# zrlhahaha/Direct12PBRRenderer

Measured on AMD Instinct MI355X. Metric: shaded Mpixel/s at 4K G-buffer (full deferred frame: clustered shade + bloom + auto-exposure + ACES), higher is better.
Workload: dtype f32

## Files before the change

direct12pbrrenderer_amd/csrc/bloom.hip:

```cpp
#include <type_traits>
#include "pbr_internal.hpp"
#include "pbr_device.hpp"

using namespace pbr;

__constant__ float c_gauss[9] = {0.0148f, 0.0459f, 0.1050f, 0.1941f, 0.2803f, 0.1941f, 0.1050f, 0.0459f, 0.0148f};

__device__ __forceinline__ float4 to4(F4 v) { return make_float4(v.x, v.y, v.z, v.w); }
__device__ __forceinline__ F4 from4(float4 v) { return f4(v.x, v.y, v.z, v.w); }

struct OutRect { int x0, y0, x1, y1, ox, oy, pitch; };
constexpr int PF_MAX_RECTS = 5;
struct OutRects {
    int n, ox, oy, pitch;
    int x0[PF_MAX_RECTS], y0[PF_MAX_RECTS], x1[PF_MAX_RECTS], y1[PF_MAX_RECTS], tiles_x[PF_MAX_RECTS], first[PF_MAX_RECTS + 1];
};
__device__ __forceinline__ float4 soft_knee_sample(F4 c, float threshold, float knee) {
    const float brightness = fmaxf(c.x, fmaxf(c.y, c.z));
    float soft = fminf(fmaxf(brightness - threshold + threshold * knee, 0.0f), 2.0f * threshold * knee);
    soft /= 4.0f * threshold * knee + 0.00001f;
    const float contribution = fmaxf(soft, brightness - threshold) / fmaxf(brightness, 0.00001f);
    const float cr = c.x * contribution, cg = c.y * contribution, cb = c.z * contribution;
    const float wgt = 1.0f / (luminance(cr, cg, cb) + 1.0f);
    return make_float4(cr * wgt, cg * wgt, cb * wgt, wgt);
// ... 377 lines not shown
    static_assert(SR % NW == 0 && TH % NW == 0 && PER_T * 8 <= 64, "rows must split evenly over the waves; one halo tap per lane");
    __shared__ float4 sLine[DUAL ? 2 : 1][NW][SW];
    __shared__ H4 sT[SR][TW];
    __shared__ uint32_t sh_hist[TAIL == 2 ? NW : 1][TAIL == 2 ? PBR_HISTOGRAM_BINS : 1];
    const int t = threadIdx.x, lane = t & 63;
    const int wv = __builtin_amdgcn_readfirstlane(t >> 6);
    if (TAIL == 2) hist_clear<NT>(sh_hist, t);
    const LevelAlpha alpha = level_alpha<MODE, DUAL>(in, iw, ih, in2, ow, oh, tr);
    for (int tile = blockIdx.x; tile < n_tiles; tile += gridDim.x) {
    const int x0 = (tr.tx0 + tile % tiles_x) * TW, y0 = (tr.ty0 + tile / tiles_x) * TH;
    const int x = x0 + lane;
    H4 hdr_in[PER_O];
    const bool in_mx = TAIL != 0 && merge_has_x(tr, x);
    if (TAIL != 0) {
#pragma unroll
        for (int k = 0; k < PER_O; k++) {
            const int y = y0 + wv + NW * k;
            if (merge_has(tr, in_mx, y)) hdr_in[k] = *reinterpret_cast<const H4*>(out + 4 * ((size_t)(y - tr.by) * out_pitch + (x - tr.bx)));
        }
    }
    const int r0 = wv * PER_T;
    const bool has_halo = lane < PER_T * 8;
    const int hk = lane >> 3, hc = 64 + (lane & 7);
    float4* line = sLine[0][wv];
    float4* line2 = sLine[DUAL ? 1 : 0][wv];
    {
        Tap2 htap;
        H4 up[DUAL ? PER_T : 1], hup;
        float fx, hfx, hfy = 0.0f;
        float4 smp[PER_T];
        int ax0, ax1, bx0, bx1;
        tap1d<MODE>(x0 - 4 + lane, iw, ax0, ax1, fx);
        tap1d<MODE>(x0 - 4 + hc, iw, bx0, bx1, hfx);
        const int sx = clampi(x0 - 4 + lane, 0, ow - 1), shx = clampi(x0 - 4 + hc, 0, ow - 1);
        const int first = y0 - 4 + r0;
        const bool shared_rows = MODE == M_UP && first >= 1 && first + PER_T - 1 <= oh - 2;
        if (MODE == M_UP && shared_rows) {
            constexpr int NR = PER_T / 2 + 2;
            const int base = (first >> 1) - 1 + (first & 1);
            V3 hrow[NR];
            const float wx0 = 1.0f - fx;
#pragma unroll
            for (int j = 0; j < NR; j++) {
                const H4* row = reinterpret_cast<const H4*>(in) + (size_t)min(base + j, ih - 1) * iw;
                const H4 c0 = row[ax0], c1 = row[ax1];
                hrow[j] = fma3(h3f(c1), fx, h3f(c0) * wx0);
            }
            auto blend = [&](auto parity) {
                constexpr int P = decltype(parity)::value;
#pragma unroll
                for (int k = 0; k < PER_T; k++) {
                    const int odd = (P + k) & 1;
                    const int i0 = (P + k + 1) / 2 - P;
                    const float fyk = odd ? 0.25f : 0.75f, wy0 = 1.0f - fyk;
                    const V3 r = fma3(hrow[i0 + 1], fyk, hrow[i0] * wy0);
                    smp[k] = make_float4(r.x, r.y, r.z, 0.0f);
                }
            };
            if (first & 1) blend(std::integral_constant<int, 1>{}); else blend(std::integral_constant<int, 0>{});
#pragma unroll
            for (int k = 0; k < PER_T; k++)
                if (DUAL) up[k] = reinterpret_cast<const H4*>(in2)[(size_t)(first + k) * ow + sx];
        } else {
            Tap2 taps[PER_T];
            float fy[PER_T];
#pragma unroll
            for (int k = 0; k < PER_T; k++) {
                const int jj = clampi(first + k, 0, oh - 1);
                int ay0, ay1;
                tap1d<MODE>(jj, ih, ay0, ay1, fy[k]);
                taps[k] = load_tap2<MODE>(in, iw, ax0, ax1, ay0, ay1);
                if (DUAL) up[k] = reinterpret_cast<const H4*>(in2)[(size_t)jj * ow + sx];
            }
#pragma unroll
            for (int k = 0; k < PER_T; k++) smp[k] = finish_tap2_rgb<MODE>(taps[k], fx, fy[k]);
        }
        if (has_halo) {
            const int jj = clampi(first + hk, 0, oh - 1);
            int ay0, ay1;
            tap1d<MODE>(jj, ih, ay0, ay1, hfy);
            htap = load_tap2<MODE>(in, iw, bx0, bx1, ay0, ay1);
            if (DUAL) hup = reinterpret_cast<const H4*>(in2)[(size_t)jj * ow + shx];
        }
#pragma unroll
        for (int k = 0; k < PER_T; k++) {
            line[lane] = smp[k];
            if (DUAL) line2[lane] = make_float4((float)up[k].x, (float)up[k].y, (float)up[k].z, 0.0f);
            if (has_halo && hk == k) {
                line[hc] = finish_tap2_rgb<MODE>(htap, hfx, hfy);
                if (DUAL) line2[hc] = make_float4((float)hup.x, (float)hup.y, (float)hup.z, 0.0f);
            }
            wave_sync();
            V3 g = gauss9_rgb(line + lane);
            if (DUAL) g = g + gauss9_rgb(line2 + lane);
            wave_sync();
            H4 th;
            th.x = to_half_rn(g.x); th.y = to_half_rn(g.y); th.z = to_half_rn(g.z); th.w = alpha.t;
            sT[r0 + k][lane] = th;
        }
    }
    __syncthreads();
#pragma unroll
    for (int k = 0; k < PER_O; k++) {
        const int r = wv + NW * k, y = y0 + r;
        if (x >= ow || y >= oh) continue;
        V3 a3 = v3(0.0f, 0.0f, 0.0f);
#pragma unroll
        for (int i = 0; i < 9; i++) a3 = fma3(h3f(sT[r + i][lane]), c_gauss[i], a3);
        const F4 a = f4(a3.x, a3.y, a3.z, alpha.v);
        if (TAIL == 0) {
            store_h4(out + 4 * ((size_t)y * out_pitch + x), a);
        } else {
            if (!(merge_has(tr, in_mx, y))) continue;
            H4 o;
            merge_rounded(a, hdr_in[k], o);
            *reinterpret_cast<H4*>(out + 4 * ((size_t)(y - tr.by) * out_pitch + (x - tr.bx))) = o;
            if (TAIL == 2) {
                if (hist_has(tr, x, y))
                    atomicAdd(&sh_hist[wv][luminance_bin_exact((float)o.x, (float)o.y, (float)o.z, min_log, inv_range)], 1u);
            }
        }
    }
    if (tile + (int)gridDim.x < n_tiles) __syncthreads();
    }
    if (TAIL == 2) {
        __syncthreads();
        hist_flush<NT>(sh_hist, t, hist);
    }
}

__device__ __forceinline__ H4 ld_h4(const void* base, uint32_t byte_off) {
    return *reinterpret_cast<const H4*>(reinterpret_cast<const char*>(base) + byte_off);
}
__device__ __forceinline__ void gauss9_pair(const float2* e, float& ge, float& go) {
    const float s[10] = {e[0].x, e[0].y, e[1].x, e[1].y, e[2].x, e[2].y, e[3].x, e[3].y, e[4].x, e[4].y};
    float a = 0.0f, b = 0.0f;
#pragma unroll
    for (int i = 0; i < 9; i++) { a = __builtin_fmaf(s[i], c_gauss[i], a); b = __builtin_fmaf(s[i + 1], c_gauss[i], b); }
    ge = a; go = b;
}

namespace poly {
constexpr double G[9] = {0.0148, 0.0459, 0.1050, 0.1941, 0.2803, 0.1941, 0.1050, 0.0459, 0.0148};
constexpr double g(int k) { return (k < -4 || k > 4) ? 0.0 : G[k + 4]; }
constexpr float E(int j) { return (float)(0.75 * g(2 * j) + 0.25 * g(2 * j + 2) + 0.75 * g(2 * j + 1) + 0.25 * g(2 * j - 1)); }
}

template <bool DUAL, int TAIL, int TH, class VS = NoViews>
__global__ __launch_bounds__(512, 4) void k_blur_up_poly(const pbr_half* __restrict__ in_, int iw, int ih,
                                                          const pbr_half* __restrict__ in2_,
                                                          pbr_half* __restrict__ out_, int ow, int oh, int out_pitch_,
                                                          int tiles_x, int n_tiles,
                                                          TailRect tr, float min_log, float inv_range, VS vs,
                                                          uint32_t* __restrict__ hist_) {
    const auto [in, in2, out, hist, out_pitch] = level_args(vs, in_, in2_, out_, hist_, out_pitch_);
    constexpr int TW = 128, NP = TW / 2 + 4, NC = TW / 2 + 6, SR = TH + 8, NT = 512, NW = NT / 64;
    constexpr int NPAIR = TH / 2 + 5;
    constexpr int PPW = (NPAIR + NW - 1) / NW;
    constexpr int PER_O = TH / 4;
    static_assert(TH % 4 == 0 && (PPW + 1) * 6 <= 64 && 2 * PPW * 4 <= 64, "one halo entry per lane");
    __shared__ H4 sLineC[NW][NC + 2];
    __shared__ float2 sLineU[DUAL ? NW : 1][3][NP];
    __shared__ H4 sT[SR][TW];
    __shared__ uint32_t sh_hist[TAIL == 2 ? NW : 1][TAIL == 2 ? PBR_HISTOGRAM_BINS : 1];
    static_assert(sizeof(sLineC) + sizeof(sLineU) + sizeof(sT) + sizeof(sh_hist) <= 80 * 1024, "k_blur_up_poly: two blocks per CU no longer fit the LDS");
    const int t = threadIdx.x, lane = t & 63;
    const int wv = __builtin_amdgcn_readfirstlane(t >> 6);
    const int vc = t & 127, vg = __builtin_amdgcn_readfirstlane(t >> 7);
    if (TAIL == 2) hist_clear<NT>(sh_hist, t);
    const LevelAlpha alpha = level_alpha<M_UP, DUAL>(in, iw, ih, in2, ow, oh, tr);
    const float a0w = (float)to_half_rn(alpha.v);
    for (int tile = blockIdx.x; tile < n_tiles; tile += gridDim.x) {
    const int x0 = (tr.tx0 + tile % tiles_x) * TW, y0 = (tr.ty0 + tile / tiles_x) * TH;
    const int xv = x0 + vc, rbase = vg * PER_O;
    H4 hdr_in[PER_O];
    const bool in_mx = TAIL != 0 && merge_has_x(tr, xv);
    char* const hdr_row0 = reinterpret_cast<char*>(out) + (ptrdiff_t)(y0 + rbase - tr.by) * out_pitch * 8;
    const uint32_t hdr_x = (uint32_t)(xv - tr.bx) * 8u;
    const size_t hdr_pitch = (size_t)out_pitch * 8u;
    {
        const int i_first = wv * PPW;
        const int n_pairs = min(PPW, NPAIR - i_first);
        const int cb = (y0 >> 1) - 3 + i_first;
        const uint32_t ccol = (uint32_t)clampi((x0 >> 1) - 3 + lane, 0, iw - 1) * 8u;
        H4 cr[PPW + 1], chalo{};
        const int hk = lane / 6, hq = 64 + lane % 6;
        const bool has_halo = lane < 6 * (PPW + 1);
        H4 upE[DUAL ? 2 * PPW : 1], upO[DUAL ? 2 * PPW : 1], hupE{}, hupO{};
        const int uk = lane >> 2, uq = 64 + (lane & 3);
        const bool has_uhalo = DUAL && lane < 8 * PPW;
        if (n_pairs > 0) {
#pragma unroll
            for (int k = 0; k <= PPW; k++) {
                const char* row = reinterpret_cast<const char*>(in) + (size_t)clampi(cb + k, 0, ih - 1) * iw * 8u;
                cr[k] = ld_h4(row, ccol);
            }
            if (has_halo) {
                const char* row = reinterpret_cast<const char*>(in) + (size_t)clampi(cb + hk, 0, ih - 1) * iw * 8u;
                chalo = ld_h4(row, (uint32_t)clampi((x0 >> 1) - 3 + hq, 0, iw - 1) * 8u);
            }
            if (DUAL) {
                const int sxe = clampi(x0 - 4 + 2 * lane, 0, ow - 1), sxo = clampi(x0 - 3 + 2 * lane, 0, ow - 1);
#pragma unroll
                for (int k = 0; k < 2 * PPW; k++) {
                    const char* row = reinterpret_cast<const char*>(in2) + (size_t)clampi(y0 - 4 + 2 * i_first - 1 + k, 0, oh - 1) * ow * 8u;
                    upE[k] = ld_h4(row, (uint32_t)sxe * 8u); upO[k] = ld_h4(row, (uint32_t)sxo * 8u);
                }
                if (has_uhalo) {
                    const uint32_t row = (uint32_t)(clampi(y0 - 4 + 2 * i_first - 1 + uk, 0, oh - 1) * ow) * 8u;
                    hupE = ld_h4(in2, row + (uint32_t)clampi(x0 - 4 + 2 * uq, 0, ow - 1) * 8u); hupO = ld_h4(in2, row + (uint32_t)clampi(x0 - 3 + 2 * uq, 0, ow - 1) * 8u);
                }
            }
        }
        if (TAIL != 0) {
#pragma unroll
            for (int k = 0; k < PER_O; k++) {
                const int y = y0 + rbase + k;
                if (merge_has(tr, in_mx, y)) hdr_in[k] = ld_h4(hdr_row0 + k * hdr_pitch, hdr_x);
            }
        }
        if (n_pairs > 0) {
            H4* line = sLineC[wv];
            float2 (*lineU)[NP] = sLineU[DUAL ? wv : 0];
            V3 pE = v3(0.0f, 0.0f, 0.0f), pO = pE;
#pragma unroll
            for (int k = 0; k <= PPW; k++) {
                if (k > n_pairs) break;
                line[lane] = cr[k];
                if (has_halo && hk == k) line[hq] = chalo;
                wave_sync();
                V3 e[7];
#pragma unroll
                for (int j = 0; j < 7; j++) e[j] = h3f(line[lane + j]);
                wave_sync();
                constexpr float PE[6] = {poly::E(-3), poly::E(-2), poly::E(-1), poly::E(0), poly::E(1), poly::E(2)};
                V3 cE = v3(0.0f, 0.0f, 0.0f), cO = cE;
#pragma unroll
                for (int j = 0; j < 6; j++) { cE = fma3(e[j], PE[j], cE); cO = fma3(e[j + 1], PE[5 - j], cO); }
                if (k > 0) {
#pragma unroll
                    for (int half = 0; half < 2; half++) {
                        const int r = 2 * (i_first + k - 1) - 1 + half;
                        if (r < 0 || r >= SR) continue;
                        const float fy = half ? 0.75f : 0.25f, wy0 = 1.0f - fy;
                        V3 bE = fma3(cE, fy, pE * wy0), bO = fma3(cO, fy, pO * wy0);
                        if (DUAL) {
                            const int u = 2 * (k - 1) + half;
                            lineU[0][lane] = make_float2((float)upE[u].x, (float)upO[u].x); lineU[1][lane] = make_float2((float)upE[u].y, (float)upO[u].y);
                            lineU[2][lane] = make_float2((float)upE[u].z, (float)upO[u].z);
                            if (has_uhalo && uk == u) {
                                lineU[0][uq] = make_float2((float)hupE.x, (float)hupO.x); lineU[1][uq] = make_float2((float)hupE.y, (float)hupO.y);
                                lineU[2][uq] = make_float2((float)hupE.z, (float)hupO.z);
                            }
                            wave_sync();
                            V3 uE, uO;
                            gauss9_pair(lineU[0] + lane, uE.x, uO.x); gauss9_pair(lineU[1] + lane, uE.y, uO.y); gauss9_pair(lineU[2] + lane, uE.z, uO.z);
                            wave_sync();
                            bE = bE + uE; bO = bO + uO;
                        }
                        struct alignas(16) H8 { H4 a, b; } th;
                        th.a.x = to_half_rn(bE.x); th.a.y = to_half_rn(bE.y); th.a.z = to_half_rn(bE.z); th.a.w = alpha.t;
                        th.b.x = to_half_rn(bO.x); th.b.y = to_half_rn(bO.y); th.b.z = to_half_rn(bO.z); th.b.w = alpha.t;
                        *reinterpret_cast<H8*>(&sT[r][2 * lane]) = th;
                    }
                }
                pE = cE; pO = cO;
            }
        }
    }
    __syncthreads();
    {
        H4 win[PER_O + 8];
#pragma unroll
        for (int i = 0; i < PER_O + 8; i++) win[i] = sT[rbase + i][vc];
#pragma unroll
        for (int k = 0; k < PER_O; k++) {
            const int y = y0 + rbase + k;
            if (xv >= ow || y >= oh) continue;
            V3 a3 = v3(0.0f, 0.0f, 0.0f);
#pragma unroll
            for (int i = 0; i < 9; i++) a3 = fma3(h3f(win[k + i]), c_gauss[i], a3);
            const F4 a = f4(a3.x, a3.y, a3.z, alpha.v);
            if (TAIL == 0) {
                store_h4(out + 4 * ((size_t)y * out_pitch + xv), a);
            } else {
                if (!(merge_has(tr, in_mx, y))) continue;
                const H4Packed o = merge_rounded_packed(a3, a0w, h4f(hdr_in[k]));
                *reinterpret_cast<H4Packed*>(hdr_row0 + k * hdr_pitch + hdr_x) = o;
                if (TAIL == 2) {
                    if (hist_has(tr, xv, y))
                        atomicAdd(&sh_hist[wv][luminance_bin_exact((float)o.lo.x, (float)o.lo.y, (float)o.hi.x, min_log, inv_range)], 1u);
                }
            }
        }
    }
    if (tile + (int)gridDim.x < n_tiles) __syncthreads();
    }
    if (TAIL == 2) {
        __syncthreads();
        hist_flush<NT>(sh_hist, t, hist);
    }
}

template <bool DUAL>
static pbr_status launch_blur_h(pbr_ctx* ctx, const pbr_half* in, uint32_t iw, uint32_t ih, const pbr_half* in2, uint32_t iw2, uint32_t ih2,
                                pbr_half* out, uint32_t ow, uint32_t oh) {
    const uint64_t row_blocks = (uint64_t)((ow + 255) / 256) * oh;
    int rows = (int)(row_blocks / 2048);
    rows = rows < 1 ? 1 : (rows > HB_MAX_ROWS ? HB_MAX_ROWS : rows);
    hipLaunchKernelGGL(k_blur_h<DUAL>, dim3((ow + 255) / 256, (oh + rows - 1) / rows), dim3(256), 0, ctx->stream, in, (int)iw, (int)ih, in2, (int)iw2, (int)ih2,
                       out, (int)ow, (int)oh, 1.0f / (float)ow, 1.0f / (float)oh, rows);
    return launched(ctx, DUAL ? "k_blur_h<dual>" : "k_blur_h");
}

static bool exact_half(uint32_t n) { return (n & 1u) == 0u && n <= 8192u; }

static TailRect tail_rect(uint32_t ow, uint32_t oh, const uint32_t* rect, const uint32_t* merge_rect, const uint32_t* buf_origin) {
    TailRect tr{};
    if (rect) { tr.hx0 = (int)rect[0]; tr.hy0 = (int)rect[1]; tr.hx1 = (int)(rect[0] + rect[2]); tr.hy1 = (int)(rect[1] + rect[3]); }
    tr.mx1 = (int)ow; tr.my1 = (int)oh;
    if (merge_rect) {
        tr.mx0 = (int)merge_rect[0]; tr.my0 = (int)merge_rect[1];
        tr.mx1 = (int)(merge_rect[0] + merge_rect[2]); tr.my1 = (int)(merge_rect[1] + merge_rect[3]);
    }
    if (buf_origin) { tr.bx = (int)buf_origin[0]; tr.by = (int)buf_origin[1]; }
    return tr;
}
struct TileGrid { int tx0, ty0, tiles_x, n; };
static TileGrid tile_grid(const TailRect& tr, int tw, int th) {
    const int tx0 = tr.mx0 / tw, ty0 = tr.my0 / th, tiles_x = (tr.mx1 + tw - 1) / tw - tx0;
    return TileGrid{tx0, ty0, tiles_x, tiles_x * ((tr.my1 + th - 1) / th - ty0)};
}

template <int MODE, bool DUAL, int TAIL, bool MV = false>
static pbr_status launch_hv(pbr_ctx* ctx, const LevelViews& lv, uint32_t nv, uint32_t iw, uint32_t ih, uint32_t ow, uint32_t oh,
                            const uint32_t* rect, float min_log, float inv_range,
                            const uint32_t* merge_rect = nullptr, const uint32_t* buf_origin = nullptr) {
    using VS = std::conditional_t<MV, LevelViews, NoViews>;
    VS vs{};
    if constexpr (MV) vs = lv;
    TailRect tr = tail_rect(ow, oh, rect, merge_rect, buf_origin);
    static const int hist_blocks = pbr::knob_int("PBR_BLOOM_HIST_BLOCKS", 1024);
    auto even_blocks = [nv](int n_tiles) { const int per = (n_tiles * (int)nv + hist_blocks - 1) / hist_blocks; return (n_tiles + per - 1) / per; };
    auto launch = [&](auto kernel, const TileGrid& g, const char* label) {
        tr.tx0 = g.tx0; tr.ty0 = g.ty0;
        hipLaunchKernelGGL(kernel, dim3(TAIL == 2 ? even_blocks(g.n) : g.n, nv), dim3(512), 0, ctx->stream,
                           MV ? nullptr : lv.in[0], (int)iw, (int)ih, MV ? nullptr : lv.in2[0], MV ? nullptr : lv.out[0], (int)ow, (int)oh,
                           MV ? 0 : lv.out_pitch[0], g.tiles_x, g.n, tr, min_log, inv_range, vs, MV ? nullptr : lv.hist[0]);
        return launched(ctx, label);
    };
    if constexpr (MODE == M_UP) {
        static const int wide_forced = pbr::knob_int("PBR_BLOOM_WIDE", -1);
        const TileGrid wide = tile_grid(tr, 128, 32);
        if (wide_forced >= 0 ? wide_forced == 1 : (wide.n >= 400 && !ctx->bloom_shader_order))
            return launch(k_blur_up_poly<DUAL, TAIL, 32, VS>, wide, MV ? "k_blur_up_poly<views>" : "k_blur_up_poly");
    }
    const TileGrid tall = tile_grid(tr, 64, 32);
    if (tall.n >= 900) return launch(k_blur_hv<MODE, DUAL, TAIL, 32, 512, VS>, tall, MV ? "k_blur_hv/32<views>" : "k_blur_hv/32");
    return launch(k_blur_hv<MODE, DUAL, TAIL, 16, 512, VS>, tile_grid(tr, 64, 16), MV ? "k_blur_hv/16<views>" : "k_blur_hv/16");
}

struct LevelIO { const pbr_half* in; const pbr_half* in2; pbr_half* out; int out_pitch; uint32_t* hist; };
template <class F>
static LevelViews level_views(uint32_t n, F io) {
    LevelViews lv{};
    for (uint32_t i = 0; i < n; i++) {
        const LevelIO v = io(i);
        lv.in[i] = v.in; lv.in2[i] = v.in2; lv.out[i] = v.out; lv.out_pitch[i] = v.out_pitch; lv.hist[i] = v.hist;
    }
    return lv;
}

static OutRects out_rects(const OutRect* rcs, int n) {
    OutRects rs{};
    rs.n = n; rs.ox = rcs[0].ox; rs.oy = rcs[0].oy; rs.pitch = rcs[0].pitch;
    int blocks = 0;
    for (int r = 0; r < n; r++) {
        rs.x0[r] = rcs[r].x0; rs.y0[r] = rcs[r].y0; rs.x1[r] = rcs[r].x1; rs.y1[r] = rcs[r].y1;
        rs.tiles_x[r] = (rcs[r].x1 - rcs[r].x0 + PF_TW - 1) / PF_TW;
        rs.first[r] = blocks;
        blocks += rs.tiles_x[r] * ((rcs[r].y1 - rcs[r].y0 + PF_TH - 1) / PF_TH);
    }
    rs.first[n] = blocks;
    return rs;
}

static pbr_status prefilter_launch(pbr_ctx* ctx, const pbr_half* hdr, uint32_t w, uint32_t h, uint32_t pitch,
                                   pbr_half* out, const OutRect* rcs, int n, float threshold, float knee) {
    const uint32_t ow = w >> 1, oh = h >> 1;
    const float tx = 1.0f / (float)ow, ty = 1.0f / (float)oh;
    if (exact_half(w) && exact_half(h)) {
        const OutRects rs = out_rects(rcs, n);
        hipLaunchKernelGGL(k_bloom_prefilter_2x<NoViews>, dim3(rs.first[n]), dim3(256), 0, ctx->stream, hdr, (int)w, (int)h, (int)pitch, NoViews{}, out, rs, threshold, knee);
        return launched(ctx, "k_bloom_prefilter_2x");
    }
    for (int r = 0; r < n; r++) {
        const uint32_t rw = (uint32_t)(rcs[r].x1 - rcs[r].x0), rh = (uint32_t)(rcs[r].y1 - rcs[r].y0);
        dim3 grid((rw + 63) / 64, (rh + 3) / 4);
        hipLaunchKernelGGL(k_bloom_prefilter, grid, dim3(64, 4), 0, ctx->stream, hdr, (int)w, (int)h, (int)pitch, out, rcs[r], tx, ty, threshold, knee);
        pbr_status st = launched(ctx, "k_bloom_prefilter");
        if (st) return st;
    }
    return PBR_OK;
}

static const char* prefilter_image_fault(uint32_t w, uint32_t h, uint32_t pitch) {
    return (w >> 1) >= 1 && (h >> 1) >= 1 && w <= 65535 && h <= 65535 && pitch >= w ? nullptr : "bad size";
}
static const char* prefilter_rect_fault(const uint32_t q[4], uint32_t w, uint32_t h, uint32_t out_x, uint32_t out_pitch) {
    if (!(q[2] >= 1 && q[3] >= 1 && q[0] + q[2] <= (w >> 1) && q[1] + q[3] <= (h >> 1))) return "rect outside the half-res image";
    return out_pitch >= out_x + q[0] + q[2] ? nullptr : "rect does not fit the output pitch";
}
static bool prefilter_dest_ok(uint32_t out_pitch, uint32_t out_y) { return out_pitch <= 65535 && out_y <= 65535; }
static const char* chain_size_fault(uint32_t w, uint32_t h, uint32_t pitch) {
    if (!((w >> (PBR_BLOOM_MIPS - 1)) >= 1 && (h >> (PBR_BLOOM_MIPS - 1)) >= 1)) return "image too small for 5 mips";
    return w <= 65535 && h <= 65535 && pitch >= w ? nullptr : "bad size";
}

static pbr_status prefilter_rects(pbr_ctx* ctx, const pbr_half* hdr, uint32_t w, uint32_t h, uint32_t pitch, pbr_half* out, uint32_t out_pitch,
                                  uint32_t out_x, uint32_t out_y, const uint32_t (*rects)[4], uint32_t n_rects, float threshold, float knee) {
    OutRect rcs[PF_MAX_RECTS];
    for (uint32_t r = 0; r < n_rects; r++) {
        const uint32_t* q = rects[r];
        rcs[r] = OutRect{(int)q[0], (int)q[1], (int)(q[0] + q[2]), (int)(q[1] + q[3]), (int)out_x, (int)out_y, (int)out_pitch};
    }
    return prefilter_launch(ctx, hdr, w, h, pitch, out, rcs, (int)n_rects, threshold, knee);
}

extern "C" {

pbr_status pbr_bloom_prefilter(pbr_ctx* ctx, const pbr_half* hdr, uint32_t w, uint32_t h, uint32_t pitch,
                               pbr_half* out, float threshold, float knee) {
    if (!ctx) return PBR_ERR_INVALID;
    PBR_REQUIRE(ctx, hdr && out, "pbr_bloom_prefilter: null pointer");
    PBR_CHECK(ctx, "pbr_bloom_prefilter", prefilter_image_fault(w, h, pitch));
    const uint32_t whole[4] = {0, 0, w >> 1, h >> 1};
    return prefilter_rects(ctx, hdr, w, h, pitch, out, w >> 1, 0, 0, &whole, 1, threshold, knee);
}

pbr_status pbr_bloom_prefilter_rect(pbr_ctx* ctx, const pbr_half* hdr, uint32_t w, uint32_t h, uint32_t pitch,
                                    pbr_half* out, uint32_t out_pitch, uint32_t out_x, uint32_t out_y,
                                    const uint32_t rect[4], float threshold, float knee) {
    if (!ctx) return PBR_ERR_INVALID;
    PBR_REQUIRE(ctx, hdr && out && rect, "pbr_bloom_prefilter_rect: null pointer");
    PBR_CHECK(ctx, "pbr_bloom_prefilter_rect", prefilter_image_fault(w, h, pitch));
    PBR_CHECK(ctx, "pbr_bloom_prefilter_rect", prefilter_rect_fault(rect, w, h, out_x, out_pitch));
    PBR_REQUIRE(ctx, prefilter_dest_ok(out_pitch, out_y), "pbr_bloom_prefilter_rect: rect does not fit the output pitch");
    return prefilter_rects(ctx, hdr, w, h, pitch, out, out_pitch, out_x, out_y, reinterpret_cast<const uint32_t (*)[4]>(rect), 1, threshold, knee);
}

pbr_status pbr_bloom_prefilter_rects(pbr_ctx* ctx, const pbr_half* hdr, uint32_t w, uint32_t h, uint32_t pitch,
                                     pbr_half* out, uint32_t out_pitch, uint32_t out_x, uint32_t out_y,
                                     const uint32_t (*rects)[4], uint32_t n_rects, float threshold, float knee) {
    if (!ctx) return PBR_ERR_INVALID;
    PBR_REQUIRE(ctx, hdr && out && rects && n_rects >= 1 && n_rects <= (uint32_t)PF_MAX_RECTS, "pbr_bloom_prefilter_rects: null pointer / 1 .. 5 rectangles");
    PBR_CHECK(ctx, "pbr_bloom_prefilter_rects", prefilter_image_fault(w, h, pitch));
    PBR_REQUIRE(ctx, prefilter_dest_ok(out_pitch, out_y), "pbr_bloom_prefilter_rects: bad size");
    for (uint32_t r = 0; r < n_rects; r++)
        PBR_REQUIRE(ctx, !prefilter_rect_fault(rects[r], w, h, out_x, out_pitch), "pbr_bloom_prefilter_rects: rectangle outside the half-res image / the output pitch");
    return prefilter_rects(ctx, hdr, w, h, pitch, out, out_pitch, out_x, out_y, rects, n_rects, threshold, knee);
}

pbr_status pbr_blur_h(pbr_ctx* ctx, const pbr_half* in, uint32_t iw, uint32_t ih, pbr_half* out, uint32_t ow, uint32_t oh) {
    if (!ctx) return PBR_ERR_INVALID;
    PBR_REQUIRE(ctx, in && out, "pbr_blur_h: null pointer");
    PBR_REQUIRE(ctx, iw && ih && ow && oh && iw <= 65535 && ih <= 65535 && ow <= 65535 && oh <= 65535, "pbr_blur_h: bad size");
    return launch_blur_h<false>(ctx, in, iw, ih, nullptr, 0, 0, out, ow, oh);
}

pbr_status pbr_blur_v(pbr_ctx* ctx, const pbr_half* in, uint32_t iw, uint32_t ih, pbr_half* out, uint32_t ow, uint32_t oh) {
    if (!ctx) return PBR_ERR_INVALID;
    PBR_REQUIRE(ctx, in && out, "pbr_blur_v: null pointer");
    PBR_REQUIRE(ctx, iw && ih && ow && oh && iw <= 65535 && ih <= 65535 && ow <= 65535 && oh <= 65535, "pbr_blur_v: bad size");
    const float tx = 1.0f / (float)ow, ty = 1.0f / (float)oh;
    dim3 grid((ow + VT_W - 1) / VT_W, (oh + VT_R - 1) / VT_R);
    hipLaunchKernelGGL(k_blur_v, grid, dim3(VT_W, 4), 0, ctx->stream, in, (int)iw, (int)ih, out, (int)ow, (int)oh, tx, ty);
    return launched(ctx, "k_blur_v");
}

pbr_status pbr_bloom_upsample_add(pbr_ctx* ctx, const pbr_half* upper, uint32_t uw, uint32_t uh,
                                  const pbr_half* lower, uint32_t lw, uint32_t lh, pbr_half* out) {
    if (!ctx) return PBR_ERR_INVALID;
    PBR_REQUIRE(ctx, upper && lower && out, "pbr_bloom_upsample_add: null pointer");
    PBR_REQUIRE(ctx, uw && uh && lw && lh && uw <= 65535 && uh <= 65535, "pbr_bloom_upsample_add: bad size");
    return launch_blur_h<true>(ctx, lower, lw, lh, upper, uw, uh, out, uw, uh);
}

pbr_status pbr_bloom_merge(pbr_ctx* ctx, pbr_half* hdr, uint32_t pitch, const pbr_half* in, uint32_t w, uint32_t h) {
    if (!ctx) return PBR_ERR_INVALID;
    PBR_REQUIRE(ctx, hdr && in, "pbr_bloom_merge: null pointer");
    PBR_REQUIRE(ctx, w && h && w <= 65535 && h <= 65535 && pitch >= w, "pbr_bloom_merge: bad size");
    dim3 grid((w + 255) / 256, h);
    hipLaunchKernelGGL(k_bloom_merge, grid, dim3(256), 0, ctx->stream, hdr, (int)pitch, in, (int)w, (int)h);
    return launched(ctx, "k_bloom_merge");
}

pbr_status pbr_bloom_up_level(pbr_ctx* ctx, const pbr_half* upper, const pbr_half* lower, uint32_t lw, uint32_t lh,
                              pbr_half* out, uint32_t ow, uint32_t oh) {
    if (!ctx) return PBR_ERR_INVALID;
    PBR_REQUIRE(ctx, lower && out && out != lower && out != upper, "pbr_bloom_up_level: null pointer / out aliases an input");
    PBR_REQUIRE(ctx, lw >= 1 && lh >= 1 && ow == 2 * lw && oh == 2 * lh && exact_half(ow) && exact_half(oh), "pbr_bloom_up_level: out must be exactly twice lower, even, <= 8192");
    const LevelViews lv = level_views(1, [&](uint32_t) { return LevelIO{lower, upper, out, (int)ow, nullptr}; });
    if (upper) return launch_hv<M_UP, true, 0>(ctx, lv, 1, lw, lh, ow, oh, nullptr, 0.0f, 0.0f);
    return launch_hv<M_UP, false, 0>(ctx, lv, 1, lw, lh, ow, oh, nullptr, 0.0f, 0.0f);
}

}

static pbr_status bloom_final(pbr_ctx* ctx, const pbr_half* b0, pbr_half* hdr, uint32_t w, uint32_t h, uint32_t pitch,
                              const uint32_t* hist_rect, float min_log, float inv_range, uint32_t* hist256) {
    const float tx = 1.0f / (float)w, ty = 1.0f / (float)h;
    const int tiles_x = (int)((w + VT_W - 1) / VT_W), tiles_y = (int)((h + VT_R - 1) / VT_R);
    int blocks = tiles_x * tiles_y;
    if (blocks > 1280) blocks = 1280;
    if (hist256) {
        hipLaunchKernelGGL(k_blur_v_merge<true>, dim3(blocks), dim3(VT_W, 4), 0, ctx->stream, b0, (int)w, (int)h, tx, ty, hdr, (int)pitch, tiles_x, tiles_y,
                           (int)hist_rect[0], (int)hist_rect[1], (int)(hist_rect[0] + hist_rect[2]), (int)(hist_rect[1] + hist_rect[3]), min_log, inv_range, hist256);
    } else {
        hipLaunchKernelGGL(k_blur_v_merge<false>, dim3(blocks), dim3(VT_W, 4), 0, ctx->stream, b0, (int)w, (int)h, tx, ty, hdr, (int)pitch, tiles_x, tiles_y,
                           0, 0, 0, 0, 0.0f, 0.0f, (uint32_t*)nullptr);
    }
    return launched(ctx, "k_blur_v_merge");
}

static void up_pass_rects(const uint32_t merge0[4], uint32_t w, uint32_t h, uint32_t need[PBR_BLOOM_MIPS][4]) {
    int x0 = (int)merge0[0], y0 = (int)merge0[1], x1 = (int)(merge0[0] + merge0[2]), y1 = (int)(merge0[1] + merge0[3]);
    for (uint32_t l = 1; l < PBR_BLOOM_MIPS; l++) {
        const int lw = (int)(w >> l), lh = (int)(h >> l);
        x0 = (x0 - 4) / 2 - 2; y0 = (y0 - 4) / 2 - 2; x1 = (x1 + 4 + 1) / 2 + 2; y1 = (y1 + 4 + 1) / 2 + 2;
        x0 = x0 < 0 ? 0 : x0; y0 = y0 < 0 ? 0 : y0; x1 = x1 > lw ? lw : x1; y1 = y1 > lh ? lh : y1;
        need[l][0] = (uint32_t)x0; need[l][1] = (uint32_t)y0; need[l][2] = (uint32_t)(x1 - x0); need[l][3] = (uint32_t)(y1 - y0);
    }
}

struct BloomView { pbr_half* hdr; uint32_t pitch; pbr_half* A; pbr_half* B; uint32_t* hist; };

template <bool MV>
static pbr_status bloom_pass(pbr_ctx* ctx, const BloomView* v, uint32_t n, uint32_t w, uint32_t h, bool prefilter, float threshold, float knee,
                             const uint32_t* hist_rect, float min_log, float inv_range, const uint32_t* merge0 = nullptr, const uint32_t* origin = nullptr) {
    auto W = [&](uint32_t l) { return w >> l; };
    auto H = [&](uint32_t l) { return h >> l; };
    auto off = [&](uint32_t l) { return (size_t)4 * pbr_bloom_level_offset(w, h, l); };
    auto exact = [&](uint32_t l) { return exact_half(W(l)) && exact_half(H(l)); };
    pbr_status r;
    if (prefilter) {
        const OutRect whole{0, 0, (int)W(1), (int)H(1), 0, 0, (int)W(1)};
        if (MV && exact(0)) {
            PrefilterViews pv{};
            for (uint32_t i = 0; i < n; i++) { pv.hdr[i] = v[i].hdr; pv.out[i] = v[i].A + off(1); pv.pitch[i] = (int)v[i].pitch; }
            const OutRects rs = out_rects(&whole, 1);
            hipLaunchKernelGGL(k_bloom_prefilter_2x<PrefilterViews>, dim3(rs.first[1], n), dim3(256), 0, ctx->stream,
                               nullptr, (int)w, (int)h, 0, pv, nullptr, rs, threshold, knee);
            if ((r = launched(ctx, "k_bloom_prefilter_2x<views>"))) return r;
        } else {
            for (uint32_t i = 0; i < n; i++)
                if ((r = prefilter_launch(ctx, v[i].hdr, w, h, v[i].pitch, v[i].A + off(1), &whole, 1, threshold, knee))) return r;
        }
    }
    for (uint32_t k = 0; k < PBR_BLOOM_STEP; k++) {
        const uint32_t up = k + 1, lo = k + 2;
        if (exact(up)) {
            const LevelViews lv = level_views(n, [&](uint32_t i) { return LevelIO{v[i].A + off(up), nullptr, v[i].A + off(lo), (int)W(lo), nullptr}; });
            if ((r = launch_hv<M_DOWN, false, 0, MV>(ctx, lv, n, W(up), H(up), W(lo), H(lo), nullptr, 0.0f, 0.0f))) return r;
        } else {
            for (uint32_t i = 0; i < n; i++) {
                if ((r = pbr_blur_h(ctx, v[i].A + off(up), W(up), H(up), v[i].B + off(lo), W(lo), H(lo)))) return r;
                if ((r = pbr_blur_v(ctx, v[i].B + off(lo), W(lo), H(lo), v[i].A + off(lo), W(lo), H(lo)))) return r;
            }
        }
    }
    uint32_t need[PBR_BLOOM_MIPS][4];
    static const bool shrink = pbr::knob_int("PBR_BLOOM_SHRINK", 1) != 0;
    const bool use_need = merge0 != nullptr && shrink;
    if (use_need) up_pass_rects(merge0, w, h, need);
    bool res_in_b = false;
    uint32_t res_level = PBR_BLOOM_MIPS - 1;
    auto res = [&](uint32_t i) { return (const pbr_half*)(res_in_b ? v[i].B : v[i].A) + off(res_level); };
    for (int k = PBR_BLOOM_STEP - 1; k >= 0; k--) {
        const uint32_t up = (uint32_t)k + 1;
        if (exact(up)) {
            const LevelViews lv = level_views(n, [&](uint32_t i) { return LevelIO{res(i), v[i].A + off(up), v[i].B + off(up), (int)W(up), nullptr}; });
            if ((r = launch_hv<M_UP, true, 0, MV>(ctx, lv, n, W(up + 1), H(up + 1), W(up), H(up), nullptr, 0.0f, 0.0f,
                                                  use_need ? need[up] : nullptr))) return r;
            res_in_b = true;
        } else {
            for (uint32_t i = 0; i < n; i++) {
                if ((r = pbr_bloom_upsample_add(ctx, v[i].A + off(up), W(up), H(up), res(i), W(up + 1), H(up + 1), v[i].B + off(up)))) return r;
                if ((r = pbr_blur_v(ctx, v[i].B + off(up), W(up), H(up), v[i].A + off(up), W(up), H(up)))) return r;
            }
            res_in_b = false;
        }
        res_level = up;
    }
    if (exact(0)) {
        const LevelViews lv = level_views(n, [&](uint32_t i) { return LevelIO{res(i), nullptr, v[i].hdr, (int)v[i].pitch, v[i].hist}; });
        if constexpr (!MV)
            if (!v[0].hist) return launch_hv<M_UP, false, 1>(ctx, lv, 1, w >> 1, h >> 1, w, h, nullptr, 0.0f, 0.0f, merge0, origin);
        return launch_hv<M_UP, false, 2, MV>(ctx, lv, n, w >> 1, h >> 1, w, h, hist_rect, min_log, inv_range, merge0, origin);
    }
    for (uint32_t i = 0; i < n; i++) {
        if ((r = pbr_blur_h(ctx, res(i), w >> 1, h >> 1, v[i].B, w, h))) return r;
        if ((r = bloom_final(ctx, v[i].B, v[i].hdr, w, h, v[i].pitch, hist_rect, min_log, inv_range, v[i].hist))) return r;
    }
    return PBR_OK;
}

extern "C" {

static pbr_status bloom_impl(pbr_ctx* ctx, pbr_half* hdr, uint32_t w, uint32_t h, uint32_t pitch, pbr_half* A, pbr_half* B,
                             float threshold, float knee, const uint32_t* hist_rect, float min_log, float inv_range, uint32_t* hist256) {
    PBR_REQUIRE(ctx, hdr && A && B, "pbr_bloom: null pointer");
    PBR_CHECK(ctx, "pbr_bloom", chain_size_fault(w, h, pitch));
    const BloomView v{hdr, pitch, A, B, hist256};
    return bloom_pass<false>(ctx, &v, 1, w, h, true, threshold, knee, hist_rect, min_log, inv_range);
}

pbr_status pbr_bloom(pbr_ctx* ctx, pbr_half* hdr, uint32_t w, uint32_t h, uint32_t pitch,
                     pbr_half* A, pbr_half* B, float threshold, float knee) {
    if (!ctx) return PBR_ERR_INVALID;
    return bloom_impl(ctx, hdr, w, h, pitch, A, B, threshold, knee, nullptr, 0.0f, 0.0f, nullptr);
}

pbr_status pbr_bloom_histogram(pbr_ctx* ctx, pbr_half* hdr, uint32_t w, uint32_t h, uint32_t pitch,
                               pbr_half* A, pbr_half* B, float threshold, float knee,
                               const uint32_t rect[4], float min_log, float inv_range, uint32_t* hist256) {
    if (!ctx) return PBR_ERR_INVALID;
    PBR_REQUIRE(ctx, rect && hist256, "pbr_bloom_histogram: null pointer");
    PBR_REQUIRE(ctx, rect[2] >= 1 && rect[3] >= 1 && rect[0] + rect[2] <= w && rect[1] + rect[3] <= h, "pbr_bloom_histogram: rect outside the image");
    return bloom_impl(ctx, hdr, w, h, pitch, A, B, threshold, knee, rect, min_log, inv_range, hist256);
}

pbr_status pbr_bloom_histogram_views(pbr_ctx* ctx, const pbr_view* views, uint32_t n, uint32_t w, uint32_t h,
                                     float threshold, float knee, float min_log, float inv_range) {
    if (!ctx) return PBR_ERR_INVALID;
    PBR_REQUIRE(ctx, views_count_ok(views, n), "pbr_bloom_histogram_views: need 1 .. PBR_MAX_VIEWS views");
    PBR_CHECK(ctx, "pbr_bloom_histogram_views", chain_size_fault(w, h, w));
    BloomView bv[PBR_MAX_VIEWS];
    for (uint32_t i = 0; i < n; i++) {
        const pbr_view& v = views[i];
        PBR_REQUIRE(ctx, v.hdr && v.chain_a && v.chain_b && v.hist256, "pbr_bloom_histogram_views: null pointer");
        PBR_REQUIRE(ctx, v.hdr_pitch >= w, "pbr_bloom_histogram_views: bad size");
        bv[i] = BloomView{v.hdr, v.hdr_pitch, v.chain_a, v.chain_b, v.hist256};
    }
    const size_t chain_bytes = pbr_bloom_chain_texels(w, h) * 8u;
    PBR_REQUIRE(ctx, views_disjoint(views, n, 4, [&](const pbr_view& v, int k, uintptr_t& lo, uintptr_t& hi) {
                    if (k == 0) { lo = addr(v.hdr); hi = lo + ((size_t)v.hdr_pitch * (h - 1) + w) * 8u; }
                    else if (k == 1) { lo = addr(v.chain_a); hi = lo + chain_bytes; }
                    else if (k == 2) { lo = addr(v.chain_b); hi = lo + chain_bytes; }
                    else { lo = addr(v.hist256); hi = lo + PBR_HISTOGRAM_BINS * sizeof(uint32_t); } }),
                "pbr_bloom_histogram_views: two views share an HDR target, a bloom chain or a histogram");
    const uint32_t rect[4] = {0, 0, w, h};
    return bloom_pass<true>(ctx, bv, n, w, h, true, threshold, knee, rect, min_log, inv_range);
}

pbr_status pbr_bloom_tiled(pbr_ctx* ctx, pbr_half* hdr, uint32_t hdr_pitch, const uint32_t hdr_rect[4],
                           uint32_t ew, uint32_t eh, pbr_half* A, pbr_half* B, const uint32_t merge_rect[4],
                           float min_log, float inv_range, uint32_t* hist256) {
    if (!ctx) return PBR_ERR_INVALID;
    PBR_REQUIRE(ctx, hdr && hdr_rect && A && B && merge_rect, "pbr_bloom_tiled: null pointer");
    PBR_REQUIRE(ctx, !chain_size_fault(ew, eh, ew), "pbr_bloom_tiled: bad size");
    PBR_REQUIRE(ctx, hdr_rect[2] >= 1 && hdr_rect[3] >= 1 && hdr_rect[0] + hdr_rect[2] <= ew && hdr_rect[1] + hdr_rect[3] <= eh && hdr_pitch >= hdr_rect[2],
                "pbr_bloom_tiled: hdr_rect outside the extended tile");
    PBR_REQUIRE(ctx, merge_rect[2] >= 1 && merge_rect[3] >= 1 && merge_rect[0] >= hdr_rect[0] && merge_rect[1] >= hdr_rect[1] &&
                     merge_rect[0] + merge_rect[2] <= hdr_rect[0] + hdr_rect[2] && merge_rect[1] + merge_rect[3] <= hdr_rect[1] + hdr_rect[3],
                "pbr_bloom_tiled: merge_rect outside hdr_rect");
    if (!exact_half(ew) || !exact_half(eh))
        return pbr::fail(ctx, PBR_ERR_UNSUPPORTED, "pbr_bloom_tiled: the extended tile must be even and <= 8192 on a side");
    const BloomView v{hdr, hdr_pitch, A, B, hist256};
    const uint32_t origin[2] = {hdr_rect[0], hdr_rect[1]};
    return bloom_pass<false>(ctx, &v, 1, ew, eh, false, 0.0f, 0.0f, merge_rect, min_log, inv_range, merge_rect, origin);
}

}
```

Before: 18410.

## Fuse smallest bloom mip down/up passes into one tiled shared-memory kernel

Adds k_bloom_small_end, which does the last downsample blur plus one or two upsample-add-blur levels per 64x16 tile entirely in LDS, recomputing halos instead of round-tripping through global memory. It replaces several small kernel launches at the low-resolution end of the bloom chain, where launch overhead and poor occupancy dominate. The cost is redundant halo computation and heavy LDS use per block. It only applies when there is a single view, no merge rect, exact halving sizes, and the levels are small enough.

```diff
diff --git a/direct12pbrrenderer_amd/csrc/bloom.hip b/direct12pbrrenderer_amd/csrc/bloom.hip
--- a/direct12pbrrenderer_amd/csrc/bloom.hip
+++ b/direct12pbrrenderer_amd/csrc/bloom.hip
@@ -703,6 +703,145 @@
     }
 }
 
+namespace small_end {
+constexpr int NT = 512, TW = 64, TH = 16;
+constexpr int R1W = 38, R1H = 14;
+constexpr int R2W = 24, R2H = 12;
+}
+__device__ __forceinline__ V3 gauss9_h(const H4* c, int stride) {
+    V3 v = v3(0.0f, 0.0f, 0.0f);
+#pragma unroll
+    for (int i = 0; i < 9; i++) v = fma3(h3f(c[i * stride]), c_gauss[i], v);
+    return v;
+}
+template <bool DUAL>
+__device__ __forceinline__ LevelAlpha level_alpha_of(float in_w, float in2_w) {
+    float alpha_h = gauss9_const(in_w);
+    if (DUAL) alpha_h = alpha_h + gauss9_const(in2_w);
+    const h16 alpha_t = to_half_rn(alpha_h);
+    return LevelAlpha{alpha_t, gauss9_const((float)alpha_t)};
+}
+template <int MODE, int SW, int SR>
+__device__ __forceinline__ void se_sample(float4* sS, const H4* src, int spitch, int sx0, int sy0, int iw, int ih, int px0, int py0, int oh, int t) {
+    constexpr int N = SW * SR, TRIPS = (N + small_end::NT - 1) / small_end::NT;
+    Tap2 tp[TRIPS];
+    float fx[TRIPS], fy[TRIPS];
+#pragma unroll
+    for (int k = 0; k < TRIPS; k++) {
+        const int e = min(t + k * small_end::NT, N - 1);
+        const int r = e / SW, c = e - r * SW;
+        int ax0, ax1, ay0, ay1;
+        tap1d<MODE>(px0 + c, iw, ax0, ax1, fx[k]);
+        tap1d<MODE>(clampi(py0 + r, 0, oh - 1), ih, ay0, ay1, fy[k]);
+        const int o0 = (ay0 - sy0) * spitch - sx0, o1 = (ay1 - sy0) * spitch - sx0;
+        tp[k].c00 = src[o0 + ax0]; tp[k].c10 = src[o0 + ax1]; tp[k].c01 = src[o1 + ax0]; tp[k].c11 = src[o1 + ax1];
+    }
+#pragma unroll
+    for (int k = 0; k < TRIPS; k++) {
+        const int e = t + k * small_end::NT;
+        if (e < N) sS[e] = finish_tap2_rgb<MODE>(tp[k], fx[k], fy[k]);
+    }
+}
+template <int SW, int SR>
+__device__ __forceinline__ void se_second(H4* sU, const pbr_half* __restrict__ in2, int ow, int oh, int px0, int py0, int t) {
+    constexpr int N = SW * SR, TRIPS = (N + small_end::NT - 1) / small_end::NT;
+    H4 u[TRIPS];
+#pragma unroll
+    for (int k = 0; k < TRIPS; k++) {
+        const int e = min(t + k * small_end::NT, N - 1);
+        const int r = e / SW, c = e - r * SW;
+        u[k] = reinterpret_cast<const H4*>(in2)[(size_t)clampi(py0 + r, 0, oh - 1) * ow + clampi(px0 + c, 0, ow - 1)];
+    }
+#pragma unroll
+    for (int k = 0; k < TRIPS; k++) {
+        const int e = t + k * small_end::NT;
+        if (e < N) sU[e] = u[k];
+    }
+}
+template <bool DUAL, int RW, int SR>
+__device__ __forceinline__ void se_hpass(H4* sT, const float4* sS, const H4* sU, h16 alpha_t, int t) {
+    for (int e = t; e < RW * SR; e += small_end::NT) {
+        const int r = e / RW, c = e - r * RW;
+        V3 g = gauss9_rgb(sS + r * (RW + 8) + c);
+        if (DUAL) g = g + gauss9_h(sU + r * (RW + 8) + c, 1);
+        H4 th;
+        th.x = to_half_rn(g.x); th.y = to_half_rn(g.y); th.z = to_half_rn(g.z); th.w = alpha_t;
+        sT[e] = th;
+    }
+}
+template <int RW, int RH>
+__device__ __forceinline__ void se_vpass(H4* sL, const H4* sT, float alpha_v, int t) {
+    for (int e = t; e < RW * RH; e += small_end::NT) {
+        const V3 a = gauss9_h(sT + e, RW);
+        H4 o;
+        o.x = to_half_rn(a.x); o.y = to_half_rn(a.y); o.z = to_half_rn(a.z); o.w = to_half_rn(alpha_v);
+        sL[e] = o;
+    }
+}
+
+template <int DEPTH>
+__global__ __launch_bounds__(small_end::NT, 4) void k_bloom_small_end(const pbr_half* __restrict__ a_lo, int lw, int lh,
+                                                                    const pbr_half* __restrict__ a_mid,
+                                                                    pbr_half* __restrict__ out, int ow, int oh, int tiles_x) {
+    using namespace small_end;
+    static_assert(DEPTH == 1 || DEPTH == 2, "one or two levels under the tile");
+    constexpr int S0W = TW + 8, S0R = TH + 8;
+    constexpr int S1W = R1W + 8, S1R = R1H + 8, S2W = R2W + 8, S2R = R2H + 8;
+    static_assert(R1W == (TW + 8) / 2 + 2 && R1H == (TH + 8) / 2 + 2 && R2W == S1W / 2 + 1 && R2H == S1R / 2 + 1, "regions of a 64 x 16 tile");
+    constexpr int NS = S0W * S0R;
+    constexpr int NU_MID = DEPTH == 2 ? S1W * S1R : 1;
+    __shared__ float4 sS[NS];
+    __shared__ H4 sU[NS];
+    __shared__ H4 sUmid[NU_MID];
+    __shared__ H4 sT[TW * S0R];
+    __shared__ H4 sR1[R1W * R1H];
+    __shared__ H4 sR2[DEPTH == 2 ? R2W * R2H : 1];
+    static_assert(sizeof(sS) + sizeof(sU) + sizeof(sUmid) + sizeof(sT) + sizeof(sR1) + sizeof(sR2) <= 80 * 1024, "k_bloom_small_end: two blocks per CU");
+    const int t = threadIdx.x;
+    const int x0 = ((int)blockIdx.x % tiles_x) * TW, y0 = ((int)blockIdx.x / tiles_x) * TH;
+    const int r1x = (x0 >> 1) - 3, r1y = (y0 >> 1) - 3;
+    const int w4 = lw >> 1, h4 = lh >> 1;
+    const float lo_w = (float)reinterpret_cast<const H4*>(a_lo)[0].w;
+    const LevelAlpha al4 = level_alpha_of<false>(lo_w, 0.0f);
+    const LevelAlpha al3 = level_alpha_of<true>((float)to_half_rn(al4.v), lo_w);
+    if constexpr (DEPTH == 1) {
+        se_sample<M_DOWN, S1W, S1R>(sS, reinterpret_cast<const H4*>(a_lo), lw, 0, 0, lw, lh, r1x - 4, r1y - 4, h4, t);
+        se_second<S0W, S0R>(sU, a_lo, ow, oh, x0 - 4, y0 - 4, t);
+        __syncthreads();
+        se_hpass<false, R1W, S1R>(sT, sS, nullptr, al4.t, t);
+        __syncthreads();
+        se_vpass<R1W, R1H>(sR1, sT, al4.v, t);
+        __syncthreads();
+    } else {
+        const int r2x = (x0 >> 2) - 4, r2y = (y0 >> 2) - 4;
+        se_sample<M_DOWN, S2W, S2R>(sS, reinterpret_cast<const H4*>(a_lo), lw, 0, 0, lw, lh, r2x - 4, r2y - 4, h4, t);
+        se_second<S1W, S1R>(sUmid, a_lo, lw, lh, r1x - 4, r1y - 4, t);
+        se_second<S0W, S0R>(sU, a_mid, ow, oh, x0 - 4, y0 - 4, t);
+        __syncthreads();
+        se_hpass<false, R2W, S2R>(sT, sS, nullptr, al4.t, t);
+        __syncthreads();
+        se_vpass<R2W, R2H>(sR2, sT, al4.v, t);
+        __syncthreads();
+        se_sample<M_UP, S1W, S1R>(sS, sR2, R2W, r2x, r2y, w4, h4, r1x - 4, r1y - 4, lh, t);
+        __syncthreads();
+        se_hpass<true, R1W, S1R>(sT, sS, sUmid, al3.t, t);
+        __syncthreads();
+        se_vpass<R1W, R1H>(sR1, sT, al3.v, t);
+        __syncthreads();
+    }
+    const LevelAlpha al = DEPTH == 1 ? al3 : level_alpha_of<true>((float)to_half_rn(al3.v), (float)reinterpret_cast<const H4*>(a_mid)[0].w);
+    se_sample<M_UP, S0W, S0R>(sS, sR1, R1W, r1x, r1y, ow >> 1, oh >> 1, x0 - 4, y0 - 4, oh, t);
+    __syncthreads();
+    se_hpass<true, TW, S0R>(sT, sS, sU, al.t, t);
+    __syncthreads();
+    for (int e = t; e < TW * TH; e += NT) {
+        const int x = x0 + (e & (TW - 1)), y = y0 + e / TW;
+        if (x >= ow || y >= oh) continue;
+        const V3 a = gauss9_h(sT + e, TW);
+        store_h4(out + 4 * ((size_t)y * ow + x), f4(a.x, a.y, a.z, al.v));
+    }
+}
+
 template <bool DUAL>
 static pbr_status launch_blur_h(pbr_ctx* ctx, const pbr_half* in, uint32_t iw, uint32_t ih, const pbr_half* in2, uint32_t iw2, uint32_t ih2,
                                 pbr_half* out, uint32_t ow, uint32_t oh) {
@@ -958,8 +1097,27 @@
                 if ((r = prefilter_launch(ctx, v[i].hdr, w, h, v[i].pitch, v[i].A + off(1), &whole, 1, threshold, knee))) return r;
         }
     }
+    static const int small_end_knob = pbr::knob_int("PBR_BLOOM_SMALL_END", 2);
+    static const int wide_forced = pbr::knob_int("PBR_BLOOM_WIDE", -1);
+    auto takes_hv16 = [&](uint32_t l) {
+        const TailRect whole = tail_rect(W(l), H(l), nullptr, nullptr, nullptr);
+        return wide_forced != 1 && tile_grid(whole, 128, 32).n < 400 && tile_grid(whole, 64, 32).n < 900;
+    };
+    int small_end = 0;
+    if (!MV && n == 1 && merge0 == nullptr && PBR_BLOOM_STEP == 3 && exact(1) && exact(2) && exact(3) && takes_hv16(3)) {
+        small_end = small_end_knob == 2 ? (takes_hv16(2) ? 2 : 0) : (small_end_knob == 1 ? 1 : 0);
+    }
+    auto launch_small_end = [&](uint32_t l) {
+        const int tiles_x = (int)((W(l) + 63) / 64), tiles = tiles_x * (int)((H(l) + 15) / 16);
+        if (l == 3) hipLaunchKernelGGL(k_bloom_small_end<1>, dim3(tiles), dim3(small_end::NT), 0, ctx->stream, (const pbr_half*)(v[0].A + off(3)), (int)W(3), (int)H(3),
+                                       (const pbr_half*)nullptr, v[0].B + off(3), (int)W(3), (int)H(3), tiles_x);
+        else hipLaunchKernelGGL(k_bloom_small_end<2>, dim3(tiles), dim3(small_end::NT), 0, ctx->stream, (const pbr_half*)(v[0].A + off(3)), (int)W(3), (int)H(3),
+                                (const pbr_half*)(v[0].A + off(2)), v[0].B + off(2), (int)W(2), (int)H(2), tiles_x);
+        return launched(ctx, l == 3 ? "k_bloom_small_end/1" : "k_bloom_small_end/2");
+    };
     for (uint32_t k = 0; k < PBR_BLOOM_STEP; k++) {
         const uint32_t up = k + 1, lo = k + 2;
+        if (small_end && lo == PBR_BLOOM_MIPS - 1) break;
         if (exact(up)) {
             const LevelViews lv = level_views(n, [&](uint32_t i) { return LevelIO{v[i].A + off(up), nullptr, v[i].A + off(lo), (int)W(lo), nullptr}; });
             if ((r = launch_hv<M_DOWN, false, 0, MV>(ctx, lv, n, W(up), H(up), W(lo), H(lo), nullptr, 0.0f, 0.0f))) return r;
@@ -979,7 +1137,10 @@
     auto res = [&](uint32_t i) { return (const pbr_half*)(res_in_b ? v[i].B : v[i].A) + off(res_level); };
     for (int k = PBR_BLOOM_STEP - 1; k >= 0; k--) {
         const uint32_t up = (uint32_t)k + 1;
-        if (exact(up)) {
+        if (small_end && up + (uint32_t)small_end >= PBR_BLOOM_MIPS - 1) {
+            if (up + (uint32_t)small_end == PBR_BLOOM_MIPS - 1 && (r = launch_small_end(up))) return r;
+            res_in_b = true;
+        } else if (exact(up)) {
             const LevelViews lv = level_views(n, [&](uint32_t i) { return LevelIO{res(i), v[i].A + off(up), v[i].B + off(up), (int)W(up), nullptr}; });
             if ((r = launch_hv<M_UP, true, 0, MV>(ctx, lv, n, W(up + 1), H(up + 1), W(up), H(up), nullptr, 0.0f, 0.0f,
                                                   use_need ? need[up] : nullptr))) return r;
```

After: 18650, median of 6. +1.3%, better.
